# baldhat/yolov10-3D

Measured on AMD Instinct MI355X. Metric: train_images_per_sec, higher is better.
Workload: dtype bf16

## Files before the change

### include/y3d.h

```cpp
#ifndef Y3D_H
#define Y3D_H
#include <stdint.h>

#ifdef __cplusplus
extern "C" {
#endif

enum { Y3D_F32 = 0, Y3D_BF16 = 1 };
enum { Y3D_OK = 0, Y3D_ERR_INVALID = -1, Y3D_ERR_HIP = -2 };

const char* y3d_last_error(void);
int y3d_abi_version(void);
int y3d_device_info(char* name, int name_len, int* compute_units, int* lds_bytes, int* clock_khz);

int y3d_pack_weight_fwd(int dtype, const float* w_oihw, void* out, int Cout, int Cin_g, int Cin_g_pad, int kh, int kw, void* stream);
int y3d_pack_weight_dgrad(int dtype, const float* w_oihw, void* out, int Cout, int Cin_g, int groups, int kh, int kw, void* stream);
int y3d_mt_pack_weights(int dtype, const int64_t* desc, const int* chunk_tensor, const int* chunk_off, int nchunks, int chunk, void* stream);
int y3d_mt_fp8w_quantize(const int64_t* desc, const int* row_begin, int ntensors, int nrows, void* stream);
int y3d_fp8w_dequantize(const uint8_t* codes, const float* scale, float* w, int rows, int K, void* stream);
int y3d_fp8_quantize_act(const void* x, int64_t xsw, int64_t M, int C, uint8_t* q, uint8_t* s, void* stream);
int y3d_fp8_pack_weight_fwd(const uint8_t* codes, const float* scale, int rows, int Cg, uint8_t* wq, uint8_t* ws, void* stream);
int y3d_conv3x3_fp8_ok(int B, int H, int W, int Cin, int Cout, int groups);
int y3d_conv3x3_fp8_stat_rows(int B, int H, int W);
int y3d_fp8_scale_pitch(int C);
int y3d_conv3x3_fp8_fwd(const uint8_t* xq, const uint8_t* xs, int B, int H, int W, int Cin, const uint8_t* wq, const uint8_t* ws, void* y, int64_t ysw,
                        int Cout, int groups, float* stat_partials, const float* scale, const float* shift, int act, void* stream);
int y3d_fp8_quantize_grad(const void* dy, int64_t sw, const float* scale, int64_t M, int C, uint8_t* q, uint8_t* s, void* stream);
int y3d_fp8_pack_weight_dgrad(const uint8_t* codes, int Cout, int Cin, int groups, int lo, int hi, uint8_t* wq, uint8_t* ws, void* stream);
int y3d_conv3x3_fp8_dgrad_ok(int B, int H, int W, int Cin, int Cout, int groups);
int y3d_conv3x3_fp8_dgrad(const uint8_t* dyq, const uint8_t* dys, int64_t qsw, int spitch, int lo, int hi, int B, int H, int W, const uint8_t* wq, const uint8_t* ws,
                          void* dx, int64_t dxsw, int Cin, int groups, void* stream);
int y3d_conv_kpad(int dtype, int k_total);
int y3d_conv_stat_blocks(int B, int Ho, int Wo);
int y3d_conv2d_stat_rows(int dtype, int B, int H, int W, int Cin, int Cout, int groups, int kh, int kw, int stride, int pad);
enum { Y3D_OP_FWD = 0, Y3D_OP_BWD_DATA = 1, Y3D_OP_BWD_WEIGHT = 2 };
enum { Y3D_EPI_RAW = 0, Y3D_EPI_PARTIALS = 1, Y3D_EPI_AFFINE = 2, Y3D_EPI_AFFINE_RES = 3, Y3D_EPI_BIAS = 4 };
enum {
  Y3D_ROUTE_GENERIC = 0,
  Y3D_ROUTE_STREAM1X1 = 1,
  Y3D_ROUTE_SMALL = 2,
  Y3D_ROUTE_SMALL_S2 = 3,
  Y3D_ROUTE_S2_DGRAD = 4,
  Y3D_ROUTE_TILE8 = 5,
  Y3D_ROUTE_TILE16 = 6,
  Y3D_ROUTE_WIDE3_8 = 7,
  Y3D_ROUTE_WIDE3_16 = 8,
  Y3D_ROUTE_FLAT = 9,
  Y3D_ROUTE_WGRAD_SMALL = 10,
  Y3D_ROUTE_WGRAD_TILE = 11,
  Y3D_ROUTE_WGRAD_STREAM1X1 = 12
};
int y3d_conv2d_route(int dtype, int op, int epi, int B, int H, int W, int Cin, int Cout, int groups, int kh, int kw, int stride, int pad);
int y3d_conv2d_fwd(int dtype, const void* x, int64_t xsb, int64_t xsh, int64_t xsw, int B, int H, int W, int Cin,
                   const void* w_packed, const float* bias, void* y, int64_t ysw, int Ho, int Wo, int Cout, int groups,
                   int kh, int kw, int stride, int pad, float* stat_partials, void* stream);
int y3d_conv2d_fwd_affine(int dtype, const void* x, int64_t xsb, int64_t xsh, int64_t xsw, int B, int H, int W, int Cin,
                          const void* w_packed, const float* scale, const float* shift, int act, void* y, int64_t ysw, int Ho, int Wo,
                          int Cout, int groups, int kh, int kw, int stride, int pad, void* stream);
int y3d_conv2d_fwd_affine_res_ok(int dtype, int B, int H, int W, int Cin, int Cout, int groups, int kh, int kw, int stride, int pad);
int y3d_conv2d_fwd_affine_res(int dtype, const void* x, int64_t xsb, int64_t xsh, int64_t xsw, int B, int H, int W, int Cin,
                              const void* w_packed, const float* scale, const float* shift, int act, const void* res, int64_t rsw, void* y,
                              int64_t ysw, int Ho, int Wo, int Cout, int groups, int kh, int kw, int stride, int pad, void* stream);
int y3d_conv2d_bwd_data(int dtype, const void* dy, int64_t dsb, int64_t dsh, int64_t dsw, int B, int Ho, int Wo, int Cout,
                        const void* w_packed_dgrad, void* dx, int64_t xsw, int H, int W, int Cin, int groups, int kh, int kw,
                        int stride, int pad, void* stream);
int y3d_conv2d_wgrad_splits(int dtype, int B, int Ho, int Wo, int Cout, int Cin_g, int groups, int kh, int kw);
int y3d_conv2d_wgrad_plan(int dtype, int B, int H, int W, int Cin, int Cout, int groups, int kh, int kw, int stride, int pad);
int y3d_set_tile_kernels(int enable);
int y3d_set_stream1x1(int enable);
int y3d_get_stream1x1(void);
int y3d_get_tile_kernels(void);
int y3d_set_bn_wide_slabs(int enable);
int y3d_set_proj_zero_skip(int enable);
int y3d_conv2d_bwd_weight(int dtype, const void* x, int64_t xsb, int64_t xsh, int64_t xsw, int B, int H, int W, int Cin,
                          int Cin_real, const void* dy, int64_t dsw, int Ho, int Wo, int Cout, int groups, int kh, int kw,
                          int stride, int pad, float* slab, int nsplit, float* grad_oihw, int accumulate, void* stream);
int y3d_wgrad_fold(const float* slab, int nsplit, int Cout, int taps, int Cin_g, int Cin_g_real, float* grad_oihw, int accumulate,
                   void* stream);

int y3d_dw_blocks(int64_t M);
int y3d_dw_wgrad_blocks(int64_t M);
int y3d_dw_pack_weight(const float* w_oihw, float* out_taps_c, int C, int kh, int kw, void* stream);
int y3d_dwconv2d_fwd(int dtype, const void* x, int64_t xsb, int64_t xsh, int64_t xsw, int B, int H, int W, int C,
                     const float* w_packed, void* y, int64_t ysw, int Ho, int Wo, int kh, int kw, int stride, int pad,
                     float* stat_partials, void* stream);
int y3d_dwconv2d_fwd_affine(int dtype, const void* x, int64_t xsb, int64_t xsh, int64_t xsw, int B, int H, int W, int C,
                            const float* w_packed, const float* scale, const float* shift, int act, int res_mode, const void* res, int64_t rsw,
                            void* z, int64_t zsw, int Ho, int Wo, int kh, int kw, int stride, int pad, void* stream);
int y3d_dwconv2d_bwd_data(int dtype, const void* dy, int64_t dsb, int64_t dsh, int64_t dsw, int B, int Ho, int Wo, int C,
                          const float* w_packed, void* dx, int64_t xsw, int H, int W, int kh, int kw, int stride, int pad,
                          void* stream);
int y3d_dwconv2d_bwd_weight(int dtype, const void* x, int64_t xsb, int64_t xsh, int64_t xsw, int B, int H, int W, int C,
                            const void* dy, int64_t dsw, int Ho, int Wo, int kh, int kw, int stride, int pad, float* slab,
                            float* grad_oihw, int accumulate, void* stream);
int y3d_dw_wgrad_fold(const float* slab, int nblk, int C, int taps, float* grad_oihw, int accumulate, void* stream);

int y3d_bn_finalize(const float* partials, int nblk, int C, int64_t count, const float* gamma, const float* beta, float eps,
                    float momentum, float* running_mean, float* running_var, float* mean, float* invstd, float* scale,
                    float* shift, void* stream);
int y3d_bn_eval_scale(int C, const float* gamma, const float* beta, const float* running_mean, const float* running_var,
                      float eps, float* scale, float* shift, void* stream);
int y3d_bn_act_fwd(int dtype, const void* y, int64_t ysw, const float* scale, const float* shift, int act, int res_mode,
                   const void* res, int64_t rsw, void* z, int64_t zsw, int64_t P, int C, void* stream);
int y3d_bn_act_fwd_q(const void* y, int64_t ysw, const float* scale, const float* shift, int act, void* z, int64_t zsw, uint8_t* q, uint8_t* s,
                     int64_t P, int C, void* stream);
int y3d_bn_bwd_blocks(int64_t P, int C);
int y3d_bn_act_bwd_reduce(int dtype, const void* y, int64_t ysw, const void* dz, int64_t dsw, const void* res, int64_t rsw,
                          const float* scale, const float* shift, const float* mean, const float* invstd, int act,
                          int res_mode, float* partials, int64_t P, int C, void* stream);
int y3d_bn_bwd_finalize(const float* partials, int nblk, int C, int64_t count, float* dgamma, float* dbeta, int accumulate,
                        float* mean_g, float* mean_gx, void* stream);
int y3d_bn_act_bwd_apply(int dtype, const void* y, int64_t ysw, const void* dz, int64_t dsw, const void* res, int64_t rsw,
                         const float* scale, const float* shift, const float* mean, const float* invstd,
                         const float* mean_g, const float* mean_gx, int act, int res_mode, int train, void* dy, int64_t dysw,
                         void* dres, int64_t drsw, int64_t P, int C, void* stream);
int y3d_colsum_partials(int dtype, const void* x, int64_t xsw, float* partials, int64_t P, int C, void* stream);

int y3d_maxpool_fwd(int dtype, const void* x, int64_t xsb, int64_t xsh, int64_t xsw, void* y, int64_t ysw, uint8_t* argmax,
                    int B, int H, int W, int C, int k, void* stream);
int y3d_maxpool_bwd(int dtype, const void* dy, int64_t dsw, const uint8_t* argmax, void* dx, int64_t xsw, int B, int H, int W,
                    int C, int k, void* stream);
int y3d_upsample2x_fwd(int dtype, const void* x, int64_t xsb, int64_t xsh, int64_t xsw, void* y, int64_t ysw, int B, int H, int W,
                       int C, void* stream);
int y3d_upsample2x_bwd(int dtype, const void* dy, int64_t dsb, int64_t dsh, int64_t dsw, void* dx, int64_t xsw, int B, int H,
                       int W, int C, void* stream);
int y3d_copy2d(int dtype, const void* x, int64_t xsw, void* y, int64_t ysw, int64_t P, int C, void* stream);
int y3d_occupy_cus(int n, const int* flag, float* buf, int64_t nbuf, void* stream);
int y3d_add2d(int dtype, const void* a, int64_t asw, const void* b, int64_t bsw, void* y, int64_t ysw, int64_t P, int C, void* stream);
int y3d_nchw_to_nhwc(int dtype, const float* x_nchw, void* y_nhwc, int B, int C, int H, int W, int Cpad, void* stream);
int y3d_stem_im2col(int dtype, const float* x_nchw, void* out, int B, int H, int W, int Ho, int Wo, void* stream);
int y3d_stem_im2col_u8(int dtype, const uint8_t* x, int hwc, void* out, int B, int H, int W, int Ho, int Wo, void* stream);
int y3d_stem_conv_eval(const void* x, int in_mode, const float* wcol, const float* scale, const float* shift, int act, void* y, int64_t ysw,
                       int B, int H, int W, int Cout, void* stream);
int y3d_stem_conv_train_rows(int B, int H, int W);
int y3d_stem_conv_train(const void* x, int in_mode, const float* wcol, void* y, int64_t ysw, void* xcol, float* part, int B, int H, int W,
                        int Cout, void* stream);
int y3d_nhwc_to_nchw(int dtype, const void* x_nhwc, int64_t xsw, float* y_nchw, int B, int C, int H, int W, void* stream);
int y3d_proj_fwd(int dtype, const void* x, int64_t xsw, const float* w, const float* bias, void* y, int64_t ysw, int64_t P,
                 int Cin, int Cout, void* stream);
int y3d_proj_bwd_data(int dtype, const void* dy, int64_t dsw, const float* w, void* dx, int64_t xsw, int64_t P, int Cin, int Cout,
                      void* stream);
int y3d_proj_blocks(int64_t P);
int y3d_proj_bwd_weight(int dtype, const void* x, int64_t xsw, const void* dy, int64_t dsw, float* slab, float* bias_slab,
                        float* grad_w, float* grad_b, int accumulate, int64_t P, int Cin, int Cout, void* stream);
int y3d_slab_reduce(const float* slab, float* out, int nblk, int64_t n, int accumulate, void* stream);
int y3d_proj_group_fwd(int dtype, int nb, int cin, const void* x, int64_t xsw, const int* xoff, const float* const* w,
                       const float* const* b, const int* couts, void* y, int64_t ysw, int64_t P, void* stream);
int y3d_proj_group_bwd_data(int dtype, int nb, int cin, const void* dy, int64_t dsw, const int* xoff, const float* const* w,
                            const int* couts, void* dx, int64_t xsw, int64_t P, void* stream);
int y3d_proj_group_fwd_bn_mfma(int nb, int cin, const void* y_pre, int64_t ysw, const int* xoff, const float* const* w, const float* const* b,
                               const int* couts, const float* scale, const float* shift, int act, void* out, int64_t osw, int64_t P,
                               void* stream);
int y3d_proj_group_bwd_weight_bn_mfma_blocks(int64_t P);
int y3d_proj_group_bwd_weight_bn_mfma(int nb, int cin, const void* y_pre, int64_t ysw, const int* xoff, const void* dout, int64_t dsw,
                                      const int* couts, const float* scale, const float* shift, int act, float* slab, float* bslab,
                                      float* const* dw, float* const* db, int64_t P, void* stream);
int y3d_proj_group_bn_bwd_blocks(int64_t P);
int y3d_proj_group_bn_bwd(int mode, int nb, int cin, const void* y_pre, int64_t ysw, const int* xoff, const void* dout, int64_t dsw,
                          const float* const* w, const int* couts, const float* scale, const float* shift, const float* mean,
                          const float* invstd, const float* mean_g, const float* mean_gx, int act, float* partials, int nblk, void* dy,
                          int64_t dysw, int64_t P, int C, void* stream);
int y3d_proj_group_blocks(int64_t P);
int y3d_proj_group_fwd_bn(int dtype, int nb, int cin, const void* y_pre, int64_t xsw, const int* xoff, const float* const* w,
                          const float* const* b, const int* couts, const float* scale, const float* shift, int act, void* out,
                          int64_t ysw, int64_t P, void* stream);
int y3d_proj_group_bwd_weight_bn(int dtype, int nb, int cin, const void* y_pre, int64_t xsw, const int* xoff, const void* dy, int64_t dsw,
                                 const int* couts, const float* scale, const float* shift, int act, float* slab, float* bslab,
                                 float* const* dw, float* const* db, int64_t P, void* stream);
int y3d_proj_group_bwd_weight(int dtype, int nb, int cin, const void* x, int64_t xsw, const int* xoff, const void* dy, int64_t dsw,
                              const int* couts, float* slab, float* bslab, float* const* dw, float* const* db, int64_t P, void* stream);

int y3d_attn_fwd(int dtype, const void* qkv, int64_t qsw, void* out, int64_t osw, float* lse, int B, int N, int nh, int kd, int hd,
                 float scale, void* stream);
int y3d_attn_bwd(int dtype, const void* qkv, int64_t qsw, const void* out, int64_t osw, const void* dout, int64_t dsw,
                 const void* dv_extra, int64_t esw, const float* lse, float* delta, void* dqkv, int64_t gsw, int B, int N, int nh,
                 int kd, int hd, float scale, void* stream);

int y3d_tal3d_scratch_floats(int B, int n, int A, int topk);
int y3d_pad_targets(const float* rows, int nbox, int width, int B, int cap, float scale_x, float scale_y, float* out, int* n_used,
                    void* stream);
int y3d_tal3d_assign(int dtype, int nl, const void* const* maps, const int64_t* psw, const int* H, const int* W, const float* strides,
                     int B, int nc, const float* gt, int n, const float* calib, const float* mean_sizes, int topk, float alpha,
                     float beta, float gamma, int mode, float* scratch, uint8_t* fg_mask, int* target_gt_idx, float* target_scores, float* scal,
                     const int* n_used, void* stream);
int y3d_loss3d(int dtype, int nl, const void* const* maps, const int64_t* psw, void* const* grads, const int64_t* gsw, const int* H,
               const int* W, const float* strides, int B, int nc, const float* gt, int n, const uint8_t* fg_mask,
               const int* target_gt_idx, const float* target_scores, const float* scal, float w_loss2d, float w_cls, float w_depth,
               float w_offset3d, float w_size3d, float w_heading, float grad_scale, float* partials, float* items, void* stream);
int y3d_loss3d_weighted(int dtype, int nl, const void* const* maps, const int64_t* psw, void* const* grads, const int64_t* gsw, const int* H,
                        const int* W, const float* strides, int B, int nc, const float* gt, int n, const uint8_t* fg_mask,
                        const int* target_gt_idx, const float* target_scores, const float* scal, float w_loss2d, float w_cls, float w_depth,
                        float w_offset3d, float w_size3d, float w_heading, float grad_scale, float* partials, float* items,
                        const float* item_w, float* total, void* stream);
int y3d_htl_update(const float* items, float time_value, int stat_epochs, float* ring, int* count, float* init_diff, int* have_init,
                   float* weights, int* status, void* stream);

int y3d_distill_loss(int dtype, int nl, const void* const* embs, const int64_t* psw, const int* H, const int* W, int B, int C,
                     const void* teacher, int teacher_dtype, int th, int tw, int64_t tsb, int64_t tsc, int64_t tsh, int64_t tsw,
                     const float* gt, int n, const uint8_t* fg_mask, const int* target_gt_idx, const float* scal, const uint8_t* mixed,
                     int img_w, int img_h, float T, float weight, int criterion, int no_mixup, int cap, int* counts, int* idx,
                     void* rows, float* partials, float* loss, void* stream);
int y3d_distill_scatter(int dtype, const void* rows, const int* idx, const int* nrows, const float* scale, int cap, int C, void* grad,
                        int64_t sb, int64_t sh, int64_t sw, int a0, int H, int W, void* stream);

int y3d_tal2d_assign(int dtype, int nl, const void* const* maps, const int64_t* psw, const int* H, const int* W, const float* strides,
                     int B, int nc, const float* gt, int n, int topk, float alpha, float beta, float* scratch, uint8_t* fg_mask,
                     int* target_gt_idx, float* target_scores, float* scal, const int* n_used, void* stream);
int y3d_loss2d(int dtype, int nl, const void* const* maps, const int64_t* psw, void* const* grads, const int64_t* gsw, const int* H,
               const int* W, const float* strides, int B, int nc, const float* gt, int n, const uint8_t* fg_mask,
               const int* target_gt_idx, const float* target_scores, const float* scal, float w_box, float w_cls, float w_dfl,
               float grad_scale, float* partials, float* items, void* stream);
int y3d_tal2d_scratch_floats(int B, int n, int A, int topk);
int y3d_tal2d_assign_crowded(int dtype, int nl, const void* const* maps, const int64_t* psw, const int* H, const int* W, const float* strides,
                             int B, int nc, const float* gt, int n, int topk, float alpha, float beta, float* scratch, uint8_t* fg_mask,
                             int* target_gt_idx, float* target_scores, float* scal, const int* n_used, void* stream);

int y3d_topk_cells(int dtype, const void* cls, int64_t psw, int B, int HW, int nc, int K, int* out_idx, void* stream);
int y3d_patch_gather(int dtype, const void* x, int64_t xsb, int64_t xsh, int64_t xsw, const int* idx, void* out, int B, int H, int W,
                     int C, int K, int ps, void* stream);
int y3d_head3d_scatter(int dtype, const void* cls, int64_t csw, const void* reg, int64_t rsw, const int* idx, void* map, int B, int HW,
                       int nc, int no, int K, void* stream);
int y3d_head3d_decode(int dtype, int nl, const void* const* maps, const int* H, const int* W, const float* strides, int B, int nc,
                      float* y, void* stream);
int y3d_head2d_decode(int dtype, int nl, const void* const* maps, const int* H, const int* W, const float* strides, int B, int nc,
                      float* y, void* stream);
int y3d_v10_postprocess_scratch_floats(int B, int A, int nc, int max_det);
// ... 122 lines not shown
```

### yolov10-3d_amd/_lib.py

```python
from __future__ import annotations

import ctypes
import os
import re

_HERE = os.path.dirname(os.path.abspath(__file__))
LIB_PATH = os.path.join(_HERE, "liby3d_hip.so")
HEADER = os.path.join(os.path.dirname(_HERE), "include", "y3d.h")

F32, BF16 = 0, 1

_CT = {"int": ctypes.c_int, "int64_t": ctypes.c_int64, "float": ctypes.c_float, "double": ctypes.c_double}


class Y3DError(RuntimeError):
    pass


def parse_header(path: str = HEADER):
    src = open(path).read()
    src = re.sub(r"/\*.*?\*/", " ", src, flags=re.S)
    protos = {}
    for m in re.finditer(r"(const\s+char\s*\*|int)\s+(y3d_\w+)\s*\(([^;{]*?)\)\s*;", src, flags=re.S):
        ret, name, args = m.group(1), m.group(2), m.group(3).strip()
        argtypes = []
        if args and args != "void":
            for a in args.split(","):
                a = a.strip()
                if "*" in a:
                    argtypes.append(ctypes.c_void_p)
                else:
                    toks = a.split()
                    t = toks[1] if toks[0] == "const" else toks[0]
                    argtypes.append(_CT[t])
        protos[name] = (ctypes.c_char_p if "char" in ret else ctypes.c_int, argtypes)
    return protos


_PLAIN_INT = {"abi_version", "conv_kpad", "conv_stat_blocks", "conv2d_stat_rows", "conv2d_route", "conv2d_wgrad_splits", "conv2d_wgrad_plan", "set_tile_kernels", "set_stream1x1", "set_bn_wide_slabs", "set_proj_zero_skip", "get_stream1x1", "get_tile_kernels", "dw_blocks", "dw_wgrad_blocks", "bn_bwd_blocks", "proj_blocks", "proj_group_blocks", "proj_group_bn_bwd_blocks", "proj_group_bwd_weight_bn_mfma_blocks", "tal3d_scratch_floats", "tal2d_scratch_floats", "v10_postprocess_scratch_floats", "conv2d_fwd_affine_res_ok", "stem_conv_train_rows", "conv3x3_fp8_ok", "conv3x3_fp8_dgrad_ok", "conv3x3_fp8_stat_rows", "fp8_scale_pitch", "kitti_eval_max_boxes", "det_metrics_max_gts", "det_metrics_max_dets"}


class _Lib:
    def __init__(self):
        if not os.path.exists(LIB_PATH):
            raise Y3DError(
                f"{LIB_PATH} not found: build it with `python yolov10-3d_amd/csrc/build.py` "
                "(or __graft_entry__.build()). There is no CPU / PyTorch fallback for the HIP path.")
        self._dll = ctypes.CDLL(LIB_PATH)
        self.protos = parse_header()
        for name, (ret, argtypes) in self.protos.items():
            fn = getattr(self._dll, name)
            fn.restype = ret
            fn.argtypes = argtypes

    def last_error(self) -> str:
        return (self._dll.y3d_last_error() or b"").decode()

    def __getattr__(self, name):
        if name.startswith("_"):
            raise AttributeError(name)
        fn = getattr(self._dll, "y3d_" + name)
        ret = self.protos["y3d_" + name][0]
        if ret is not ctypes.c_int or name in _PLAIN_INT:
            setattr(self, name, fn)
            return fn

        def call(*a):
            rc = fn(*a)
            if rc != 0:
                raise Y3DError(f"y3d_{name} failed ({rc}): {self.last_error()}")
            return rc

        setattr(self, name, call)
        return call


_lib = None


def lib() -> _Lib:
    global _lib
    if _lib is None:
        _lib = _Lib()
    return _lib
```

### yolov10-3d_amd/csrc/proj_bn_mfma.hip

```cpp
#include "common.h"

namespace {

constexpr int PB_MAXB = 16;
int g_proj_zero_skip = 1;

struct PBP {
  const bf16_t* y;
  const bf16_t* dout;
  bf16_t* dy;
  float* part;
  const float* w[PB_MAXB];
  int xoff[PB_MAXB], ooff[PB_MAXB], cout[PB_MAXB];
  const float *scale, *shift, *mean, *invstd, *mg, *mgx;
  long ysw, dsw, dysw, P;
  int cin, C, act, px_per_block, zskip;
};

constexpr int PZ_MAXGRP = 1024;

__device__ __forceinline__ void projg_scan_dout(const bf16_t* dop, long dsw, int cout, long pbeg, long pend, int first, int ngrp,
                                                unsigned char* zact, int wave, int lane) {
  constexpr int GB = 8;
  for (int i0 = first + wave; i0 < ngrp; i0 += 4 * GB) {
    unsigned m[GB];
#pragma unroll
    for (int k = 0; k < GB; ++k) m[k] = 0;
    for (int o0 = 0, ow = 1; o0 < cout; o0 += ow, ow = 8) {
      unsigned bits[GB];
#pragma unroll
      for (int k = 0; k < GB; ++k) {
        const long px = pbeg + (long)(i0 + 4 * k) * 64 + lane;
        bits[k] = 0;
        if (i0 + 4 * k < ngrp && px < pend) {
          const bf16_t* r = dop + px * dsw + o0;
#pragma unroll
          for (int j = 0; j < 8; ++j)
            if (j < ow && o0 + j < cout) bits[k] |= r[j];
        }
      }
      bool full = true;
#pragma unroll
      for (int k = 0; k < GB; ++k) {
        const unsigned long long bm = __ballot(bits[k] != 0);
        m[k] |= ((bm & 0xFFFFull) ? 1u : 0u) | ((bm & 0xFFFF0000ull) ? 2u : 0u) | ((bm & 0xFFFF00000000ull) ? 4u : 0u) |
                ((bm & 0xFFFF000000000000ull) ? 8u : 0u);
        full = full && (m[k] == 0xFu || i0 + 4 * k >= ngrp);
      }
      if (full) break;
    }
#pragma unroll
    for (int k = 0; k < GB; ++k)
      if (lane == 0 && i0 + 4 * k < ngrp) zact[i0 + 4 * k] = (unsigned char)m[k];
  }
}

__device__ __forceinline__ int projg_scan_run(const bf16_t* dop, long dsw, int cout, long pbeg, long pend, int ngrp, unsigned char* zact,
                                              int wave, int lane) {
  if (wave == 0) projg_scan_dout(dop, dsw, cout, pbeg, pend, 0, 1, zact, 0, lane);
  __syncthreads();
  if (__builtin_amdgcn_readfirstlane((int)zact[0]) == 0xF) return 0;
  projg_scan_dout(dop, dsw, cout, pbeg, pend, 1, ngrp, zact, wave, lane);
  __syncthreads();
  return ngrp;
}

template <int MODE, int NT>
__global__ __launch_bounds__(256) void projg_bn_bwd_kernel(PBP p) {
  constexpr int CIN = NT * 16, LDW = CIN + 4;
  constexpr int CH = CIN / 8;
  constexpr int PPP = 64 / CH;
  constexpr int NPASS = 16 / PPP;
  static_assert(NPASS >= 1 && 64 % CH == 0 && 16 % PPP == 0, "cin must be 32, 64 or 128");
  extern __shared__ __attribute__((aligned(16))) float psm[];
  const int tid = threadIdx.x, lane = tid & 63, wave = tid >> 6;
  const int q = lane >> 4, lp = lane & 15;
  const int br = blockIdx.y, run = blockIdx.x, cout = p.cout[br];
  float* tile = psm + wave * 16 * LDW;

  bf16x8_t wf[NT];
  {
    const float* w = p.w[br];
#pragma unroll
    for (int t = 0; t < NT; ++t)
#pragma unroll
      for (int j = 0; j < 8; ++j) {
        const int o = 8 * q + j;
        wf[t][j] = (__bf16)(o < cout ? w[o * CIN + t * 16 + lp] : 0.f);
      }
  }
  const int cc = lane % CH, pr = lane / CH;
  const int c0 = p.xoff[br] + cc * 8;
  float sc[8], sf[8], mu[8], is[8], m1[8], m2[8], s1[8], s2[8];
#pragma unroll
  for (int j = 0; j < 8; ++j) {
    sc[j] = p.scale[c0 + j]; sf[j] = p.shift[c0 + j]; mu[j] = p.mean[c0 + j]; is[j] = p.invstd[c0 + j];
    if (MODE == 1) { m1[j] = p.mg[c0 + j]; m2[j] = p.mgx[c0 + j]; }
    s1[j] = 0.f; s2[j] = 0.f;
  }
  const long pbeg = (long)run * p.px_per_block;
  const long pend = pbeg + p.px_per_block < p.P ? pbeg + p.px_per_block : p.P;
  const bf16_t* dop = p.dout + p.ooff[br];
  __shared__ unsigned char zact[PZ_MAXGRP];
  const int nstep = pend > pbeg ? (int)((pend - pbeg + 63) >> 6) : 0;
  int nscan = (MODE == 0 && p.zskip) ? (nstep < PZ_MAXGRP ? nstep : PZ_MAXGRP) : 0;
  if (nscan) nscan = projg_scan_run(dop, p.dsw, cout, pbeg, pend, nscan, zact, __builtin_amdgcn_readfirstlane(wave), lane);
  for (long pb = pbeg; pb < pend; pb += 64) {
    const int step = (int)((pb - pbeg) >> 6);
    const unsigned m = step < nscan ? (unsigned)__builtin_amdgcn_readfirstlane((int)zact[step]) : 0xFu;
    if (m == 0) continue;
    const bool live = __builtin_amdgcn_readfirstlane((int)((m >> wave) & 1u)) != 0;
    const long p0 = pb + wave * 16;
    uint4 yv[NPASS];
    if (live) {
#pragma unroll
      for (int s = 0; s < NPASS; ++s) {
        const long px = p0 + s * PPP + pr;
        yv[s] = px < pend ? *(const uint4*)(p.y + px * p.ysw + c0) : make_uint4(0, 0, 0, 0);
      }
      bf16x8_t a;
      {
        const long px = p0 + lp;
        const bool pok = px < pend;
#pragma unroll
        for (int j = 0; j < 8; ++j) {
          const int o = 8 * q + j;
          unsigned short raw = 0;
          if (pok && o < cout) raw = dop[px * p.dsw + o];
          a[j] = __builtin_bit_cast(__bf16, raw);
        }
      }
#pragma unroll
      for (int t = 0; t < NT; ++t) {
        const f32x4_t d = __builtin_amdgcn_mfma_f32_16x16x32_bf16(a, wf[t], (f32x4_t){0.f, 0.f, 0.f, 0.f}, 0, 0, 0);
#pragma unroll
        for (int r = 0; r < 4; ++r) tile[(4 * q + r) * LDW + t * 16 + lp] = d[r];
      }
    }
    __syncthreads();
    if (live) {
#pragma unroll
      for (int s = 0; s < NPASS; ++s) {
        const int pl = s * PPP + pr;
        const long px = p0 + pl;
        const float4 z0 = *(const float4*)(tile + pl * LDW + cc * 8), z1 = *(const float4*)(tile + pl * LDW + cc * 8 + 4);
        const float dz[8] = {z0.x, z0.y, z0.z, z0.w, z1.x, z1.y, z1.z, z1.w};
        float v[8], o[8];
        Chunk<bf16_t>::unpack(yv[s], v);
#pragma unroll
        for (int j = 0; j < 8; ++j) {
          float g = dz[j];
          if (p.act) g *= silu_grad_f(v[j] * sc[j] + sf[j]);
          const float xh = (v[j] - mu[j]) * is[j];
          if (MODE == 0) { s1[j] += g; s2[j] += g * (v[j] - mu[j]) * is[j]; }
          else o[j] = sc[j] * (g - m1[j] - xh * m2[j]);
        }
        if (MODE == 1 && px < pend) *(uint4*)(p.dy + px * p.dysw + c0) = Chunk<bf16_t>::pack(o);
      }
    }
    __syncthreads();
  }
  if (MODE == 0) {
    float* red = psm;
#pragma unroll
    for (int j = 0; j < 8; ++j) {
      red[((wave * PPP + pr) * CIN + cc * 8 + j) * 2 + 0] = s1[j];
      red[((wave * PPP + pr) * CIN + cc * 8 + j) * 2 + 1] = s2[j];
    }
    __syncthreads();
    if (tid < CIN) {
      float a0 = 0.f, a1 = 0.f;
      for (int r = 0; r < 4 * PPP; ++r) { a0 += red[(r * CIN + tid) * 2]; a1 += red[(r * CIN + tid) * 2 + 1]; }
      float* dst = p.part + ((long)run * p.C + p.xoff[br] + tid) * 2;
      dst[0] = a0;
      dst[1] = a1;
    }
  }
}

struct PFP {
  const bf16_t* y;
  bf16_t* out;
  const float* w[PB_MAXB];
  const float* b[PB_MAXB];
  int xoff[PB_MAXB], ooff[PB_MAXB], cout[PB_MAXB];
  const float *scale, *shift;
  long ysw, osw, P;
  int act, px_per_block;
};

template <int NT>
__global__ __launch_bounds__(256) void projg_fwd_bn_mfma_kernel(PFP p) {
  constexpr int CIN = NT * 16, KS = CIN / 32;
  constexpr int LDB = CIN * 2 + 16;
  constexpr int CH = CIN / 8, PPP = 64 / CH, NPASS = 16 / PPP;
  extern __shared__ __attribute__((aligned(16))) float psm[];
  const int tid = threadIdx.x, lane = tid & 63, wave = tid >> 6;
  const int q = lane >> 4, lp = lane & 15;
  const int br = blockIdx.y, cout = p.cout[br];
  char* tile = (char*)psm + wave * 16 * LDB;
  bf16x8_t wf[2][KS];
  float bias[2];
  {
    const float* w = p.w[br];
#pragma unroll
    for (int n = 0; n < 2; ++n) {
      const int o = 16 * n + lp;
      bias[n] = o < cout ? p.b[br][o] : 0.f;
#pragma unroll
      for (int ks = 0; ks < KS; ++ks)
#pragma unroll
        for (int j = 0; j < 8; ++j) wf[n][ks][j] = (__bf16)(o < cout ? w[o * CIN + ks * 32 + 8 * q + j] : 0.f);
    }
  }
  const int cc = lane % CH, pr = lane / CH;
  const int c0 = p.xoff[br] + cc * 8;
  float sc[8], sf[8];
#pragma unroll
  for (int j = 0; j < 8; ++j) { sc[j] = p.scale[c0 + j]; sf[j] = p.shift[c0 + j]; }
  const long pbeg = (long)blockIdx.x * p.px_per_block;
  const long pend = pbeg + p.px_per_block < p.P ? pbeg + p.px_per_block : p.P;
  bf16_t* op = p.out + p.ooff[br];
  const bool two = cout > 16;
  for (long pb = pbeg; pb < pend; pb += 64) {
    const long p0 = pb + wave * 16;
    uint4 yv[NPASS];
#pragma unroll
    for (int s = 0; s < NPASS; ++s) {
      const long px = p0 + s * PPP + pr;
      yv[s] = px < pend ? *(const uint4*)(p.y + px * p.ysw + c0) : make_uint4(0, 0, 0, 0);
    }
#pragma unroll
    for (int s = 0; s < NPASS; ++s) {
      float v[8];
      Chunk<bf16_t>::unpack(yv[s], v);
#pragma unroll
      for (int j = 0; j < 8; ++j) {
        const float u = v[j] * sc[j] + sf[j];
        v[j] = p.act ? silu_f(u) : u;
      }
      *(uint4*)(tile + (s * PPP + pr) * LDB + cc * 16) = Chunk<bf16_t>::pack(v);
    }
    __syncthreads();
    f32x4_t acc0 = {0.f, 0.f, 0.f, 0.f}, acc1 = {0.f, 0.f, 0.f, 0.f};
#pragma unroll
    for (int ks = 0; ks < KS; ++ks) {
      const bf16x8_t a = __builtin_bit_cast(bf16x8_t, *(const uint4*)(tile + lp * LDB + (ks * 4 + q) * 16));
      acc0 = __builtin_amdgcn_mfma_f32_16x16x32_bf16(a, wf[0][ks], acc0, 0, 0, 0);
      if (two) acc1 = __builtin_amdgcn_mfma_f32_16x16x32_bf16(a, wf[1][ks], acc1, 0, 0, 0);
    }
#pragma unroll
    for (int r = 0; r < 4; ++r) {
      const long px = p0 + 4 * q + r;
      if (px < pend) {
        if (lp < cout) op[px * p.osw + lp] = f2bf(acc0[r] + bias[0]);
        if (two && 16 + lp < cout) op[px * p.osw + 16 + lp] = f2bf(acc1[r] + bias[1]);
      }
    }
    __syncthreads();
  }
}

struct PWP {
  const bf16_t* y;
  const bf16_t* dout;
  float* slab;
  float* bslab;
  float* dw[PB_MAXB];
  float* db[PB_MAXB];
  int xoff[PB_MAXB], ooff[PB_MAXB], cout[PB_MAXB];
  const float *scale, *shift;
  long ysw, dsw, P;
  int act, px_per_block, ctot, zskip;
};

template <int NT>
__global__ __launch_bounds__(256) void projg_bwd_weight_bn_mfma_kernel(PWP p) {
  constexpr int CIN = NT * 16;
  constexpr int LDB = CIN * 2 + 32;
  constexpr int CH = CIN / 8, PPP = 64 / CH, NPASS = 32 / PPP;
  extern __shared__ __attribute__((aligned(16))) float psm[];
  const int tid = threadIdx.x, lane = tid & 63, wave = tid >> 6;
  const int g = lane >> 4, lp = lane & 15;
  const int br = blockIdx.y, run = blockIdx.x, cout = p.cout[br];
  const bool two = cout > 16;
  char* tile = (char*)psm + wave * 32 * LDB;
  const int cc = lane % CH, pr = lane / CH;
  const int c0 = p.xoff[br] + cc * 8;
  float sc[8], sf[8];
#pragma unroll
  for (int j = 0; j < 8; ++j) { sc[j] = p.scale[c0 + j]; sf[j] = p.shift[c0 + j]; }
  f32x4_t acc[2][NT];
#pragma unroll
  for (int n = 0; n < 2; ++n)
#pragma unroll
    for (int t = 0; t < NT; ++t) acc[n][t] = (f32x4_t){0.f, 0.f, 0.f, 0.f};
  float bsum[2] = {0.f, 0.f};
  const long pbeg = (long)run * p.px_per_block;
  const long pend = pbeg + p.px_per_block < p.P ? pbeg + p.px_per_block : p.P;
  const bf16_t* dop = p.dout + p.ooff[br];
  const int trow = 4 * g + (lp >> 2), tcol = (lp & 3) * 4;
  __shared__ unsigned char zact[PZ_MAXGRP];
  const int ngrp = pend > pbeg ? 2 * (int)((pend - pbeg + 127) >> 7) : 0;
  int nscan = p.zskip ? (ngrp < PZ_MAXGRP ? ngrp : PZ_MAXGRP) : 0;
  if (nscan) nscan = projg_scan_run(dop, p.dsw, cout, pbeg, pend, nscan, zact, __builtin_amdgcn_readfirstlane(wave), lane);
  for (long pb = pbeg; pb < pend; pb += 128) {
    const int g0 = (int)((pb - pbeg) >> 6);
    const unsigned m = g0 < nscan ? (unsigned)__builtin_amdgcn_readfirstlane((int)zact[g0] | ((int)zact[g0 + 1] << 4)) : 0xFFu;
    if (m == 0) continue;
    const bool live = __builtin_amdgcn_readfirstlane((int)((m >> (2 * wave)) & 3u)) != 0;
    const long p0 = pb + wave * 32;
    bf16x8_t a[2];
    if (live) {
      uint4 yv[NPASS];
#pragma unroll
      for (int s = 0; s < NPASS; ++s) {
        const long px = p0 + s * PPP + pr;
        yv[s] = px < pend ? *(const uint4*)(p.y + px * p.ysw + c0) : make_uint4(0, 0, 0, 0);
      }
#pragma unroll
      for (int n = 0; n < 2; ++n)
#pragma unroll
        for (int j = 0; j < 8; ++j) {
          const long px = p0 + 16 * (j >> 2) + 4 * g + (j & 3);
          const int o = 16 * n + lp;
          unsigned short raw = 0;
          if ((n == 0 || two) && o < cout && px < pend) raw = dop[px * p.dsw + o];
          a[n][j] = __builtin_bit_cast(__bf16, raw);
          bsum[n] += bf2f(raw);
        }
#pragma unroll
      for (int s = 0; s < NPASS; ++s) {
        float v[8];
        Chunk<bf16_t>::unpack(yv[s], v);
#pragma unroll
        for (int j = 0; j < 8; ++j) {
          const float u = v[j] * sc[j] + sf[j];
          v[j] = p.act ? silu_f(u) : u;
        }
        *(uint4*)(tile + (s * PPP + pr) * LDB + cc * 16) = Chunk<bf16_t>::pack(v);
      }
    }
    __syncthreads();
    if (live) {
#pragma unroll
      for (int t = 0; t < NT; ++t) {
        const char* a0 = tile + trow * LDB + (t * 16 + tcol) * 2;
        const s16x4_t lo = __builtin_amdgcn_ds_read_tr16_b64_v4i16((s16x4_t __attribute__((address_space(3)))*)(a0));
        const s16x4_t hi = __builtin_amdgcn_ds_read_tr16_b64_v4i16((s16x4_t __attribute__((address_space(3)))*)(a0 + 16 * LDB));
        typedef __attribute__((ext_vector_type(8))) short s16x8_t;
        const bf16x8_t b = __builtin_bit_cast(bf16x8_t, (s16x8_t)__builtin_shufflevector(lo, hi, 0, 1, 2, 3, 4, 5, 6, 7));
        acc[0][t] = __builtin_amdgcn_mfma_f32_16x16x32_bf16(a[0], b, acc[0][t], 0, 0, 0);
        if (two) acc[1][t] = __builtin_amdgcn_mfma_f32_16x16x32_bf16(a[1], b, acc[1][t], 0, 0, 0);
      }
    }
    __syncthreads();
  }
  float* red = psm;
  const int NO = two ? 2 : 1;
  for (int n = 0; n < NO; ++n)
#pragma unroll
    for (int t = 0; t < NT; ++t)
#pragma unroll
      for (int r = 0; r < 4; ++r) red[(wave * 32 + 16 * n + 4 * g + r) * CIN + t * 16 + lp] = (n == 0 ? acc[0][t][r] : acc[1][t][r]);
  __shared__ float bred[4][32];
#pragma unroll
  for (int n = 0; n < 2; ++n) {
    float v = bsum[n];
    v = lane_xor32_sum(lane_xor16_sum(v));
    if (g == 0) bred[wave][16 * n + lp] = v;
  }
  __syncthreads();
  for (int i = tid; i < cout * CIN; i += 256) {
    const int o = i / CIN, ch = i - o * CIN;
    p.slab[((long)run * p.ctot + p.ooff[br] + o) * CIN + ch] =
        red[(0 * 32 + o) * CIN + ch] + red[(1 * 32 + o) * CIN + ch] + red[(2 * 32 + o) * CIN + ch] + red[(3 * 32 + o) * CIN + ch];
  }
  if (tid < cout) p.bslab[(long)run * p.ctot + p.ooff[br] + tid] = bred[0][tid] + bred[1][tid] + bred[2][tid] + bred[3][tid];
}

__device__ __forceinline__ float slab_sum_in_order(const float* __restrict__ src, long pitch, int nblk) {
  float s = 0.f;
  int b = 0;
  for (; b + 8 <= nblk; b += 8) {
    float v[8];
#pragma unroll
    for (int j = 0; j < 8; ++j) v[j] = src[(long)(b + j) * pitch];
#pragma unroll
    for (int j = 0; j < 8; ++j) s += v[j];
  }
  for (; b < nblk; ++b) s += src[(long)b * pitch];
  return s;
}

__global__ void projg_wslab_reduce_kernel(PWP p, int nblk, int cin) {
  const int br = blockIdx.y, cout = p.cout[br];
  const int idx = blockIdx.x * blockDim.x + threadIdx.x;
  if (idx < cout * cin) p.dw[br][idx] = slab_sum_in_order(p.slab + (long)p.ooff[br] * cin + idx, (long)p.ctot * cin, nblk);
  if (idx < cout) p.db[br][idx] = slab_sum_in_order(p.bslab + p.ooff[br] + idx, p.ctot, nblk);
}

}

extern "C" {

int y3d_set_proj_zero_skip(int enable) {
  const int old = g_proj_zero_skip;
  g_proj_zero_skip = enable ? 1 : 0;
  return old;
}

int y3d_proj_group_bwd_weight_bn_mfma_blocks(int64_t P) {
  long n = (P + 1023) / 1024;
  return (int)(n < 1 ? 1 : (n > 64 ? 64 : n));
}

int y3d_proj_group_bwd_weight_bn_mfma(int nb, int cin, const void* y_pre, int64_t ysw, const int* xoff, const void* dout, int64_t dsw,
                                      const int* couts, const float* scale, const float* shift, int act, float* slab, float* bslab,
                                      float* const* dw, float* const* db, int64_t P, void* stream) {
  Y3D_CHECK(nb >= 1 && nb <= PB_MAXB && (cin == 64 || cin == 128), "proj_group_bwd_weight_bn_mfma: 1..16 branches of 64 or 128 channels");
  Y3D_CHECK(y_pre && dout && scale && shift && slab && bslab && dw && db && P >= 1 && ysw % 8 == 0 && ((uintptr_t)y_pre & 15) == 0,
            "proj_group_bwd_weight_bn_mfma: null / misaligned argument");
  PWP p;
  p.y = (const bf16_t*)y_pre; p.dout = (const bf16_t*)dout; p.slab = slab; p.bslab = bslab;
  int off = 0;
  for (int i = 0; i < nb; ++i) {
    Y3D_CHECK(couts[i] >= 1 && couts[i] <= 32 && xoff[i] % 8 == 0, "proj_group_bwd_weight_bn_mfma: cout in 1..32, channel slices 16-byte aligned");
    p.dw[i] = dw[i]; p.db[i] = db[i]; p.xoff[i] = xoff[i]; p.ooff[i] = off; p.cout[i] = couts[i];
    off += couts[i];
  }
  Y3D_CHECK(dsw >= off, "proj_group_bwd_weight_bn_mfma: dout pixel stride smaller than the projected channels");
  p.scale = scale; p.shift = shift; p.ysw = ysw; p.dsw = dsw; p.P = P; p.act = act; p.ctot = off; p.zskip = g_proj_zero_skip;
  const int nrun = y3d_proj_group_bwd_weight_bn_mfma_blocks(P);
  p.px_per_block = (int)(((P + nrun - 1) / nrun + 127) / 128 * 128);
  hipStream_t st = (hipStream_t)stream;
  const size_t sm = (size_t)4 * 32 * cin * sizeof(float);
  static bool attr = false;
  if (!attr) {
    (void)hipFuncSetAttribute((const void*)projg_bwd_weight_bn_mfma_kernel<8>, hipFuncAttributeMaxDynamicSharedMemorySize, 4 * 32 * 128 * 4);
    (void)hipFuncSetAttribute((const void*)projg_bwd_weight_bn_mfma_kernel<4>, hipFuncAttributeMaxDynamicSharedMemorySize, 4 * 32 * 64 * 4);
    attr = true;
  }
  if (cin == 128) hipLaunchKernelGGL((projg_bwd_weight_bn_mfma_kernel<8>), dim3(nrun, nb), dim3(256), sm, st, p);
  else hipLaunchKernelGGL((projg_bwd_weight_bn_mfma_kernel<4>), dim3(nrun, nb), dim3(256), sm, st, p);
  hipLaunchKernelGGL(projg_wslab_reduce_kernel, dim3((32 * cin + 255) / 256, nb), dim3(256), 0, st, p, nrun, cin);
  Y3D_LAUNCH_CHECK();
  return Y3D_OK;
}

int y3d_proj_group_fwd_bn_mfma(int nb, int cin, const void* y_pre, int64_t ysw, const int* xoff, const float* const* w, const float* const* b,
                               const int* couts, const float* scale, const float* shift, int act, void* out, int64_t osw, int64_t P,
                               void* stream) {
  Y3D_CHECK(nb >= 1 && nb <= PB_MAXB && (cin == 64 || cin == 128), "proj_group_fwd_bn_mfma: 1..16 branches of 64 or 128 channels");
  Y3D_CHECK(y_pre && out && w && b && scale && shift && P >= 1 && ysw % 8 == 0 && ((uintptr_t)y_pre & 15) == 0, "proj_group_fwd_bn_mfma: null / misaligned argument");
  PFP p;
  p.y = (const bf16_t*)y_pre; p.out = (bf16_t*)out;
  int off = 0;
  for (int i = 0; i < nb; ++i) {
    Y3D_CHECK(couts[i] >= 1 && couts[i] <= 32 && xoff[i] % 8 == 0, "proj_group_fwd_bn_mfma: cout in 1..32, channel slices 16-byte aligned");
    p.w[i] = w[i]; p.b[i] = b[i]; p.xoff[i] = xoff[i]; p.ooff[i] = off; p.cout[i] = couts[i];
    off += couts[i];
  }
  Y3D_CHECK(osw >= off, "proj_group_fwd_bn_mfma: output pixel stride smaller than the projected channels");
  p.scale = scale; p.shift = shift; p.ysw = ysw; p.osw = osw; p.P = P; p.act = act;
  long nrun = (P + 63) / 64;
  if (nrun > 128) nrun = 128;
  p.px_per_block = (int)(((P + nrun - 1) / nrun + 63) / 64 * 64);
  dim3 grid((unsigned)nrun, nb);
  hipStream_t st = (hipStream_t)stream;
  if (cin == 128) hipLaunchKernelGGL((projg_fwd_bn_mfma_kernel<8>), grid, dim3(256), (size_t)4 * 16 * (128 * 2 + 16), st, p);
  else hipLaunchKernelGGL((projg_fwd_bn_mfma_kernel<4>), grid, dim3(256), (size_t)4 * 16 * (64 * 2 + 16), st, p);
  Y3D_LAUNCH_CHECK();
  return Y3D_OK;
}

int y3d_proj_group_bn_bwd_blocks(int64_t P) {
  long n = (P + 63) / 64;
  return (int)(n < 1 ? 1 : (n > 128 ? 128 : n));
}

int y3d_proj_group_bn_bwd(int mode, int nb, int cin, const void* y_pre, int64_t ysw, const int* xoff, const void* dout, int64_t dsw,
                          const float* const* w, const int* couts, const float* scale, const float* shift, const float* mean,
                          const float* invstd, const float* mean_g, const float* mean_gx, int act, float* partials, int nblk, void* dy,
                          int64_t dysw, int64_t P, int C, void* stream) {
  Y3D_CHECK(mode == 0 || mode == 1, "proj_group_bn_bwd: mode 0 (reduce) or 1 (apply)");
  Y3D_CHECK(nb >= 1 && nb <= PB_MAXB && (cin == 64 || cin == 128), "proj_group_bn_bwd: 1..16 branches of 64 or 128 channels");
  Y3D_CHECK(y_pre && dout && scale && shift && mean && invstd && P >= 1, "proj_group_bn_bwd: null argument");
  Y3D_CHECK(mode == 0 ? (partials != nullptr && nblk == y3d_proj_group_bn_bwd_blocks(P)) : (dy && mean_g && mean_gx && dysw >= cin),
            "proj_group_bn_bwd: partials / nblk (reduce) or dy / mean_g / mean_gx (apply) missing");
  Y3D_CHECK(ysw % 8 == 0 && ((uintptr_t)y_pre & 15) == 0 && (mode == 0 || (dysw % 8 == 0 && ((uintptr_t)dy & 15) == 0)), "proj_group_bn_bwd: 16-byte alignment");
  PBP p;
  p.y = (const bf16_t*)y_pre; p.dout = (const bf16_t*)dout; p.dy = (bf16_t*)dy; p.part = partials;
  int off = 0;
  for (int i = 0; i < nb; ++i) {
    Y3D_CHECK(couts[i] >= 1 && couts[i] <= 32 && xoff[i] % 8 == 0 && xoff[i] + cin <= C, "proj_group_bn_bwd: cout in 1..32, channel slices 16-byte aligned inside C");
    p.w[i] = w[i]; p.xoff[i] = xoff[i]; p.ooff[i] = off; p.cout[i] = couts[i];
    off += couts[i];
  }
  Y3D_CHECK(dsw >= off, "proj_group_bn_bwd: dout pixel stride smaller than the projected channels");
  p.scale = scale; p.shift = shift; p.mean = mean; p.invstd = invstd; p.mg = mean_g; p.mgx = mean_gx;
  p.ysw = ysw; p.dsw = dsw; p.dysw = dysw; p.P = P; p.cin = cin; p.C = C; p.act = act; p.zskip = g_proj_zero_skip;
  const int nrun = y3d_proj_group_bn_bwd_blocks(P);
  p.px_per_block = (int)(((P + nrun - 1) / nrun + 63) / 64 * 64);
  dim3 grid(nrun, nb);
  hipStream_t st = (hipStream_t)stream;
  const size_t sm128 = (size_t)4 * 16 * (128 + 4) * sizeof(float), sm64 = (size_t)4 * 16 * (64 + 4) * sizeof(float);
  if (cin == 128) {
    if (mode == 0) hipLaunchKernelGGL((projg_bn_bwd_kernel<0, 8>), grid, dim3(256), sm128, st, p);
    else hipLaunchKernelGGL((projg_bn_bwd_kernel<1, 8>), grid, dim3(256), sm128, st, p);
  } else {
    if (mode == 0) hipLaunchKernelGGL((projg_bn_bwd_kernel<0, 4>), grid, dim3(256), sm64, st, p);
    else hipLaunchKernelGGL((projg_bn_bwd_kernel<1, 4>), grid, dim3(256), sm64, st, p);
  }
  Y3D_LAUNCH_CHECK();
  return Y3D_OK;
}

}
```

Measured before the change: 1445.

## Double-buffer global loads in projected-group BN backward stats kernel

Result: no change. 1450, median of 4 (+0.3%).

```diff
diff --git a/include/y3d.h b/include/y3d.h
--- a/include/y3d.h
+++ b/include/y3d.h
@@ -72,6 +72,7 @@
 int y3d_get_tile_kernels(void);
 int y3d_set_bn_wide_slabs(int enable);
 int y3d_set_proj_zero_skip(int enable);
+int y3d_set_proj_pipeline(int enable);
 int y3d_conv2d_bwd_weight(int dtype, const void* x, int64_t xsb, int64_t xsh, int64_t xsw, int B, int H, int W, int Cin,
                           int Cin_real, const void* dy, int64_t dsw, int Ho, int Wo, int Cout, int groups, int kh, int kw,
                           int stride, int pad, float* slab, int nsplit, float* grad_oihw, int accumulate, void* stream);
diff --git a/yolov10-3d_amd/_lib.py b/yolov10-3d_amd/_lib.py
--- a/yolov10-3d_amd/_lib.py
+++ b/yolov10-3d_amd/_lib.py
@@ -37,7 +37,7 @@
     return protos
 
 
-_PLAIN_INT = {"abi_version", "conv_kpad", "conv_stat_blocks", "conv2d_stat_rows", "conv2d_route", "conv2d_wgrad_splits", "conv2d_wgrad_plan", "set_tile_kernels", "set_stream1x1", "set_bn_wide_slabs", "set_proj_zero_skip", "get_stream1x1", "get_tile_kernels", "dw_blocks", "dw_wgrad_blocks", "bn_bwd_blocks", "proj_blocks", "proj_group_blocks", "proj_group_bn_bwd_blocks", "proj_group_bwd_weight_bn_mfma_blocks", "tal3d_scratch_floats", "tal2d_scratch_floats", "v10_postprocess_scratch_floats", "conv2d_fwd_affine_res_ok", "stem_conv_train_rows", "conv3x3_fp8_ok", "conv3x3_fp8_dgrad_ok", "conv3x3_fp8_stat_rows", "fp8_scale_pitch", "kitti_eval_max_boxes", "det_metrics_max_gts", "det_metrics_max_dets"}
+_PLAIN_INT = {"abi_version", "conv_kpad", "conv_stat_blocks", "conv2d_stat_rows", "conv2d_route", "conv2d_wgrad_splits", "conv2d_wgrad_plan", "set_tile_kernels", "set_stream1x1", "set_bn_wide_slabs", "set_proj_zero_skip", "set_proj_pipeline","get_stream1x1", "get_tile_kernels", "dw_blocks", "dw_wgrad_blocks", "bn_bwd_blocks", "proj_blocks", "proj_group_blocks", "proj_group_bn_bwd_blocks", "proj_group_bwd_weight_bn_mfma_blocks", "tal3d_scratch_floats", "tal2d_scratch_floats", "v10_postprocess_scratch_floats", "conv2d_fwd_affine_res_ok", "stem_conv_train_rows", "conv3x3_fp8_ok", "conv3x3_fp8_dgrad_ok", "conv3x3_fp8_stat_rows", "fp8_scale_pitch", "kitti_eval_max_boxes", "det_metrics_max_gts", "det_metrics_max_dets"}
 
 
 class _Lib:
diff --git a/yolov10-3d_amd/csrc/proj_bn_mfma.hip b/yolov10-3d_amd/csrc/proj_bn_mfma.hip
--- a/yolov10-3d_amd/csrc/proj_bn_mfma.hip
+++ b/yolov10-3d_amd/csrc/proj_bn_mfma.hip
@@ -1,9 +1,11 @@
 #include "common.h"
+#include "proj_pipeline_sched.h"
 
 namespace {
 
 constexpr int PB_MAXB = 16;
 int g_proj_zero_skip = 1;
+int g_proj_pipeline = 1;
 
 struct PBP {
   const bf16_t* y;
@@ -65,8 +67,9 @@
   return ngrp;
 }
 
-template <int MODE, int NT>
-__global__ __launch_bounds__(256) void projg_bn_bwd_kernel(PBP p) {
+template <int MODE, int NT, bool PIPE>
+__device__ __forceinline__ void projg_bn_bwd_body(const PBP& p) {
+  static_assert(MODE == 0 || !PIPE, "the apply pass keeps the serial loop");
   constexpr int CIN = NT * 16, LDW = CIN + 4;
   constexpr int CH = CIN / 8;
   constexpr int PPP = 64 / CH;
@@ -78,8 +81,11 @@
   const int br = blockIdx.y, run = blockIdx.x, cout = p.cout[br];
   float* tile = psm + wave * 16 * LDW;
 
+  const int cc = lane % CH, pr = lane / CH;
+  const int c0 = p.xoff[br] + cc * 8;
   bf16x8_t wf[NT];
-  {
+  float sc[8], sf[8], mu[8], is[8], m1[8], m2[8], s1[8], s2[8];
+  auto load_consts = [&]() __attribute__((always_inline)) {
     const float* w = p.w[br];
 #pragma unroll
     for (int t = 0; t < NT; ++t)
@@ -88,16 +94,15 @@
         const int o = 8 * q + j;
         wf[t][j] = (__bf16)(o < cout ? w[o * CIN + t * 16 + lp] : 0.f);
       }
-  }
-  const int cc = lane % CH, pr = lane / CH;
-  const int c0 = p.xoff[br] + cc * 8;
-  float sc[8], sf[8], mu[8], is[8], m1[8], m2[8], s1[8], s2[8];
-#pragma unroll
-  for (int j = 0; j < 8; ++j) {
-    sc[j] = p.scale[c0 + j]; sf[j] = p.shift[c0 + j]; mu[j] = p.mean[c0 + j]; is[j] = p.invstd[c0 + j];
-    if (MODE == 1) { m1[j] = p.mg[c0 + j]; m2[j] = p.mgx[c0 + j]; }
-    s1[j] = 0.f; s2[j] = 0.f;
-  }
+#pragma unroll
+    for (int j = 0; j < 8; ++j) {
+      sc[j] = p.scale[c0 + j]; sf[j] = p.shift[c0 + j]; mu[j] = p.mean[c0 + j]; is[j] = p.invstd[c0 + j];
+      if (MODE == 1) { m1[j] = p.mg[c0 + j]; m2[j] = p.mgx[c0 + j]; }
+    }
+  };
+#pragma unroll
+  for (int j = 0; j < 8; ++j) { s1[j] = 0.f; s2[j] = 0.f; }
+  if (!PIPE) load_consts();
   const long pbeg = (long)run * p.px_per_block;
   const long pend = pbeg + p.px_per_block < p.P ? pbeg + p.px_per_block : p.P;
   const bf16_t* dop = p.dout + p.ooff[br];
@@ -105,31 +110,45 @@
   const int nstep = pend > pbeg ? (int)((pend - pbeg + 63) >> 6) : 0;
   int nscan = (MODE == 0 && p.zskip) ? (nstep < PZ_MAXGRP ? nstep : PZ_MAXGRP) : 0;
   if (nscan) nscan = projg_scan_run(dop, p.dsw, cout, pbeg, pend, nscan, zact, __builtin_amdgcn_readfirstlane(wave), lane);
-  for (long pb = pbeg; pb < pend; pb += 64) {
-    const int step = (int)((pb - pbeg) >> 6);
-    const unsigned m = step < nscan ? (unsigned)__builtin_amdgcn_readfirstlane((int)zact[step]) : 0xFu;
-    if (m == 0) continue;
-    const bool live = __builtin_amdgcn_readfirstlane((int)((m >> wave) & 1u)) != 0;
-    const long p0 = pb + wave * 16;
-    uint4 yv[NPASS];
-    if (live) {
+  auto mask = [&](int step) __attribute__((always_inline)) -> unsigned { return step < nscan ? (unsigned)__builtin_amdgcn_readfirstlane((int)zact[step]) : 0xFu; };
+  auto fetch = [&](int step, uint4(&yv)[NPASS], unsigned short(&raw)[8]) __attribute__((always_inline)) {
+    if (__builtin_amdgcn_readfirstlane((int)((mask(step) >> wave) & 1u)) == 0) return;
+    const long p0 = pbeg + (long)step * 64 + __builtin_amdgcn_readfirstlane(wave) * 16;
+    if constexpr (PIPE) {
+      const char* yb = (const char*)(p.y + p0 * p.ysw + p.xoff[br]);
+      const unsigned ylane = (unsigned)((pr * p.ysw + cc * 8) * 2);
+#pragma unroll
+      for (int s = 0; s < NPASS; ++s)
+        yv[s] = p0 + s * PPP + pr < pend ? *(const uint4*)(yb + (long)s * PPP * p.ysw * 2 + ylane) : make_uint4(0, 0, 0, 0);
+    } else {
 #pragma unroll
       for (int s = 0; s < NPASS; ++s) {
         const long px = p0 + s * PPP + pr;
         yv[s] = px < pend ? *(const uint4*)(p.y + px * p.ysw + c0) : make_uint4(0, 0, 0, 0);
       }
+    }
+    const long px = p0 + lp;
+    const bool pok = px < pend;
+    const bf16_t* row = dop + (pok ? px : pend - 1) * p.dsw;
+#pragma unroll
+    for (int j = 0; j < 8; ++j) {
+      const int o = 8 * q + j;
+      raw[j] = 0;
+      if constexpr (PIPE) {
+        if (j < cout) raw[j] = row[o < cout ? o : j];
+      } else {
+        if (pok && o < cout) raw[j] = dop[px * p.dsw + o];
+      }
+    }
+  };
+  auto compute = [&](int step, const uint4(&yv)[NPASS], const unsigned short(&raw)[8]) __attribute__((always_inline)) {
+    const bool live = __builtin_amdgcn_readfirstlane((int)((mask(step) >> wave) & 1u)) != 0;
+    const long p0 = pbeg + (long)step * 64 + wave * 16;
+    if (live) {
       bf16x8_t a;
-      {
-        const long px = p0 + lp;
-        const bool pok = px < pend;
-#pragma unroll
-        for (int j = 0; j < 8; ++j) {
-          const int o = 8 * q + j;
-          unsigned short raw = 0;
-          if (pok && o < cout) raw = dop[px * p.dsw + o];
-          a[j] = __builtin_bit_cast(__bf16, raw);
-        }
-      }
+      const bool pok = p0 + lp < pend;
+#pragma unroll
+      for (int j = 0; j < 8; ++j) a[j] = __builtin_bit_cast(__bf16, (unsigned short)(pok && 8 * q + j < cout ? raw[j] : 0));
 #pragma unroll
       for (int t = 0; t < NT; ++t) {
         const f32x4_t d = __builtin_amdgcn_mfma_f32_16x16x32_bf16(a, wf[t], (f32x4_t){0.f, 0.f, 0.f, 0.f}, 0, 0, 0);
@@ -159,6 +178,49 @@
       }
     }
     __syncthreads();
+  };
+  if constexpr (PIPE) {
+    uint4 yv[PROJP_DEPTH][NPASS];
+    unsigned short a[PROJP_DEPTH][8];
+    const int first = projp_next_active(mask, nstep, 0);
+    if (first >= nstep) {
+      if (tid < CIN) {
+        float* dst = p.part + ((long)run * p.C + p.xoff[br] + tid) * 2;
+        dst[0] = 0.f;
+        dst[1] = 0.f;
+      }
+      return;
+    }
+    fetch(first, yv[0], a[0]);
+    load_consts();
+#pragma unroll
+    for (int j = 0; j < 8; ++j) asm volatile("" ::"v"(sc[j]), "v"(sf[j]), "v"(mu[j]), "v"(is[j]));
+#pragma unroll
+    for (int t = 0; t < NT; ++t) asm volatile("" ::"v"(wf[t]));
+    projp_walk_from(
+        mask, nstep, first,
+        [&](int step, auto st, int) __attribute__((always_inline)) {
+#pragma unroll
+          for (int s = 0; s < NPASS; ++s) {
+            const uint4 v = yv[decltype(st)::value][s];
+            asm volatile("" ::"v"(v.x), "v"(v.y), "v"(v.z), "v"(v.w));
+          }
+#pragma unroll
+          for (int j = 0; j < 8; ++j) {
+            const unsigned r = a[decltype(st)::value][j];
+            asm volatile("" ::"v"(r));
+          }
+        },
+        [&](int step, auto st) __attribute__((always_inline)) { fetch(step, yv[decltype(st)::value], a[decltype(st)::value]); },
+        [&](int step, auto st, int) __attribute__((always_inline)) { compute(step, yv[decltype(st)::value], a[decltype(st)::value]); });
+  } else {
+    uint4 yv[NPASS];
+    unsigned short a[8];
+    for (int step = 0; step < nstep; ++step) {
+      if (mask(step) == 0) continue;
+      fetch(step, yv, a);
+      compute(step, yv, a);
+    }
   }
   if (MODE == 0) {
     float* red = psm;
@@ -176,6 +238,16 @@
       dst[1] = a1;
     }
   }
+}
+
+template <int MODE, int NT>
+__global__ __launch_bounds__(256) __attribute__((amdgpu_waves_per_eu((MODE == 1 ? 3 : 2) + (NT == 4 ? 1 : 0)))) void projg_bn_bwd_kernel(PBP p) {
+  projg_bn_bwd_body<MODE, NT, MODE == 0>(p);
+}
+
+template <int NT>
+__global__ __launch_bounds__(256) void projg_bn_bwd_serial_kernel(PBP p) {
+  projg_bn_bwd_body<0, NT, false>(p);
 }
 
 struct PFP {
@@ -410,6 +482,12 @@
   return old;
 }
 
+int y3d_set_proj_pipeline(int enable) {
+  const int old = g_proj_pipeline;
+  g_proj_pipeline = enable ? 1 : 0;
+  return old;
+}
+
 int y3d_proj_group_bwd_weight_bn_mfma_blocks(int64_t P) {
   long n = (P + 1023) / 1024;
   return (int)(n < 1 ? 1 : (n > 64 ? 64 : n));
@@ -506,10 +584,12 @@
   hipStream_t st = (hipStream_t)stream;
   const size_t sm128 = (size_t)4 * 16 * (128 + 4) * sizeof(float), sm64 = (size_t)4 * 16 * (64 + 4) * sizeof(float);
   if (cin == 128) {
-    if (mode == 0) hipLaunchKernelGGL((projg_bn_bwd_kernel<0, 8>), grid, dim3(256), sm128, st, p);
+    if (mode == 0 && g_proj_pipeline) hipLaunchKernelGGL((projg_bn_bwd_kernel<0, 8>), grid, dim3(256), sm128, st, p);
+    else if (mode == 0) hipLaunchKernelGGL((projg_bn_bwd_serial_kernel<8>), grid, dim3(256), sm128, st, p);
     else hipLaunchKernelGGL((projg_bn_bwd_kernel<1, 8>), grid, dim3(256), sm128, st, p);
   } else {
-    if (mode == 0) hipLaunchKernelGGL((projg_bn_bwd_kernel<0, 4>), grid, dim3(256), sm64, st, p);
+    if (mode == 0 && g_proj_pipeline) hipLaunchKernelGGL((projg_bn_bwd_kernel<0, 4>), grid, dim3(256), sm64, st, p);
+    else if (mode == 0) hipLaunchKernelGGL((projg_bn_bwd_serial_kernel<4>), grid, dim3(256), sm64, st, p);
     else hipLaunchKernelGGL((projg_bn_bwd_kernel<1, 4>), grid, dim3(256), sm64, st, p);
   }
   Y3D_LAUNCH_CHECK();
diff --git a/yolov10-3d_amd/csrc/proj_pipeline_sched.h b/yolov10-3d_amd/csrc/proj_pipeline_sched.h
--- /dev/null
+++ b/yolov10-3d_amd/csrc/proj_pipeline_sched.h
@@ -0,0 +1,58 @@
+#pragma once
+
+#if defined(__HIPCC__) || defined(__CUDACC__)
+#define PROJP_HD __host__ __device__ __forceinline__
+#else
+#define PROJP_HD inline
+#endif
+
+constexpr int PROJP_DEPTH = 2;
+
+template <int S>
+struct projp_stage_c {
+  static constexpr int value = S;
+};
+
+template <class Mask>
+PROJP_HD int projp_next_active(const Mask& mask, int nstep, int from) {
+  while (from < nstep && mask(from) == 0) ++from;
+  return from;
+}
+
+PROJP_HD int projp_stage(int k) { return k % PROJP_DEPTH; }
+
+PROJP_HD int projp_ahead(int left) { return left < PROJP_DEPTH - 1 ? left : PROJP_DEPTH - 1; }
+
+PROJP_HD int projp_behind() { return 0; }
+
+template <class Mask, class Ready, class Fetch, class Use>
+PROJP_HD void projp_walk_from(const Mask& mask, int nstep, int first, Ready&& ready, Fetch&& fetch, Use&& use) {
+  static_assert(PROJP_DEPTH == 2, "the walk is written out for two stages");
+  int cur = first;
+  for (;;) {
+    {
+      const int nxt = projp_next_active(mask, nstep, cur + 1);
+      ready(cur, projp_stage_c<0>{}, projp_behind());
+      if (nxt < nstep) fetch(nxt, projp_stage_c<1>{});
+      use(cur, projp_stage_c<0>{}, projp_ahead(nxt < nstep ? 1 : 0));
+      if (nxt >= nstep) return;
+      cur = nxt;
+    }
+    {
+      const int nxt = projp_next_active(mask, nstep, cur + 1);
+      ready(cur, projp_stage_c<1>{}, projp_behind());
+      if (nxt < nstep) fetch(nxt, projp_stage_c<0>{});
+      use(cur, projp_stage_c<1>{}, projp_ahead(nxt < nstep ? 1 : 0));
+      if (nxt >= nstep) return;
+      cur = nxt;
+    }
+  }
+}
+
+template <class Mask, class Ready, class Fetch, class Use>
+PROJP_HD void projp_walk(const Mask& mask, int nstep, Ready&& ready, Fetch&& fetch, Use&& use) {
+  const int first = projp_next_active(mask, nstep, 0);
+  if (first >= nstep) return;
+  fetch(first, projp_stage_c<0>{});
+  projp_walk_from(mask, nstep, first, ready, fetch, use);
+}
```
